# WUTCM-Lab/GLSDet

Hardware: AMD Instinct MI355X
Metric: images/sec fwd @1333x800 bs=8 (detection forward incl. decode+NMS) (higher is better)
Workload: dtype f16; 1 GPU; yolox_s_glfusion_1344x800_bs8; detector=YOLOX-s + GL-fusion neck, images_per_gpu=8, global_batch=8, num_classes=10, hip_graph=True, batches_in_flight=3, parallelism=image-sharded dp1, one all_gather of detections per step

## Files before the change

### glsdet_amd/_lib.py

```python
import ctypes as C
import threading
import os

HERE = os.path.dirname(os.path.abspath(__file__))
LIB_PATH = os.path.join(HERE, "lib", "libglsdet_hip.so")
ABI_VERSION = 13
CAPTURE_LOCK = threading.RLock()

F16, F32 = 0, 1
ACT = {"none": 0, "silu": 1, "relu": 2, "lrelu": 3, "gelu": 4, "sigmoid": 5}


class GlsdetLibraryError(RuntimeError):
    pass


class GlsdetError(RuntimeError):
    """A C-ABI call returned a negative code; nothing was launched."""


class View(C.Structure):
    _fields_ = [("base", C.c_void_p), ("sn", C.c_int64), ("sh", C.c_int64), ("sw", C.c_int64),
                ("n", C.c_int32), ("h", C.c_int32), ("w", C.c_int32), ("c", C.c_int32),
                ("dtype", C.c_int32), ("_pad", C.c_int32),
                ("alloc_lo", C.c_void_p), ("alloc_hi", C.c_void_p)]


class ConvDesc(C.Structure):
    _fields_ = [("x", View), ("y", View), ("res", View),
                ("w", C.c_void_p), ("scale", C.c_void_p), ("bias", C.c_void_p),
                ("R", C.c_int32), ("S", C.c_int32), ("stride", C.c_int32), ("pad", C.c_int32),
                ("act", C.c_int32), ("tile_hint", C.c_int32)]


class ConvChain(C.Structure):
    _fields_ = [("y2", View), ("w2", C.c_void_p), ("scale2", C.c_void_p), ("bias2", C.c_void_p),
                ("act2", C.c_int32), ("c0", C.c_int32), ("cin2", C.c_int32), ("flags", C.c_int32)]


_SIGS = {
    "glsdet_conv2d_chain": (C.c_int, [C.POINTER(ConvDesc), C.POINTER(ConvChain), C.c_void_p]),
    "glsdet_conv2d_chain_tune": (C.c_int, [C.POINTER(ConvDesc), C.POINTER(ConvChain), C.c_void_p, C.POINTER(C.c_int32),
                                           C.POINTER(C.c_float)]),
    "glsdet_conv2d_gnstats_bytes": (C.c_int64, [C.c_int32, C.c_int32, C.c_int32, C.c_int32]),
    "glsdet_conv2d_gnstats": (C.c_int, [C.POINTER(ConvDesc), C.c_int32, C.c_void_p, C.c_void_p]),
    "glsdet_conv2d_gnstats_tune": (C.c_int, [C.POINTER(ConvDesc), C.c_int32, C.c_void_p, C.c_void_p, C.POINTER(C.c_int32),
                                             C.POINTER(C.c_float)]),
    "glsdet_bottleneck": (C.c_int, [C.POINTER(ConvDesc), C.POINTER(ConvDesc), C.c_int32, C.c_void_p]),
    "glsdet_bottleneck_tune": (C.c_int, [C.POINTER(ConvDesc), C.POINTER(ConvDesc), C.c_void_p, C.POINTER(C.c_int32),
                                         C.POINTER(C.c_float)]),
    "glsdet_conv2d": (C.c_int, [C.POINTER(ConvDesc), C.c_void_p]),
    "glsdet_conv2d_multi": (C.c_int, [C.POINTER(ConvDesc), C.c_int32, C.c_void_p]),
    "glsdet_conv2d_multi_tune": (C.c_int, [C.POINTER(ConvDesc), C.c_int32, C.c_void_p, C.POINTER(C.c_int32),
                                           C.POINTER(C.c_float)]),
    "glsdet_conv2d_tune": (C.c_int, [C.POINTER(ConvDesc), C.c_void_p, C.POINTER(C.c_int32), C.POINTER(C.c_float)]),
    "glsdet_dwconv2d": (C.c_int, [C.POINTER(ConvDesc), C.c_void_p]),
    "glsdet_dwconv2d_dilated": (C.c_int, [C.POINTER(ConvDesc), C.c_int32, C.c_void_p]),
    "glsdet_gate": (C.c_int, [C.POINTER(View), C.POINTER(View), C.POINTER(View), C.POINTER(View), C.c_int32, C.c_void_p]),
    "glsdet_conv_weight_elems": (C.c_int64, [C.c_int32] * 5),
    "glsdet_conv_kpad": (C.c_int32, [C.c_int32] * 4),
    "glsdet_conv_cout_pad": (C.c_int32, [C.c_int32]),
    "glsdet_focus_pack": (C.c_int, [C.c_void_p, C.c_int32, C.c_int32, C.c_int32, C.c_int32,
                                    C.POINTER(View), C.c_void_p]),
    "glsdet_focus_conv": (C.c_int, [C.c_void_p, C.c_int32, C.c_int32, C.c_int32, C.c_int32, C.c_void_p, C.c_void_p, C.c_void_p,
                                    C.c_int32, C.POINTER(View), C.c_void_p]),
    "glsdet_focus_conv_down": (C.c_int, [C.c_void_p, C.c_int32, C.c_int32, C.c_int32, C.c_int32, C.c_void_p, C.c_void_p, C.c_void_p,
                                         C.c_int32, C.c_int32, C.c_void_p, C.c_void_p, C.c_void_p, C.c_int32, C.POINTER(View),
                                         C.c_void_p]),
    "glsdet_resnet_stem_weight_elems": (C.c_int64, []),
    "glsdet_resnet_stem_pool": (C.c_int, [C.c_void_p, C.c_int32, C.c_int32, C.c_int32, C.c_int32, C.c_void_p, C.c_void_p, C.c_void_p,
                                          C.POINTER(View), C.c_void_p]),
    "glsdet_resnet_stem": (C.c_int, [C.c_void_p, C.c_int32, C.c_int32, C.c_int32, C.c_int32, C.c_void_p, C.c_void_p, C.c_void_p,
                                     C.c_int32, C.POINTER(View), C.c_void_p]),
    "glsdet_channel_maxmean": (C.c_int, [C.POINTER(View), C.POINTER(View), C.c_void_p]),
    "glsdet_spp_pools": (C.c_int, [C.POINTER(View), C.POINTER(View), C.POINTER(View), C.POINTER(View), C.c_void_p]),
    "glsdet_maxpool2d": (C.c_int, [C.POINTER(View), C.POINTER(View), C.c_int32, C.c_void_p]),
    "glsdet_resample_copy": (C.c_int, [C.POINTER(View), C.POINTER(View), C.c_int32, C.c_void_p]),
    "glsdet_copy_many": (C.c_int, [C.POINTER(View), C.POINTER(View), C.c_int32, C.c_void_p]),
    "glsdet_transpose_many": (C.c_int, [C.POINTER(View), C.POINTER(View), C.c_int32, C.c_void_p]),
    "glsdet_nonlocal": (C.c_int, [C.POINTER(View), C.POINTER(View), C.c_int32, C.c_void_p, C.c_void_p,
                                  C.c_void_p, C.POINTER(View), C.c_void_p]),
    "glsdet_nonlocal_multi": (C.c_int, [C.POINTER(View), C.POINTER(View), C.c_int32, C.c_int32, C.POINTER(C.c_void_p),
                                        C.POINTER(C.c_void_p), C.c_void_p, C.POINTER(View), C.c_void_p]),
    "glsdet_attn_split": (C.c_int, [C.POINTER(View), C.c_void_p, C.c_void_p]),
    "glsdet_nonlocal_split": (C.c_int, [C.POINTER(View), C.POINTER(View), C.c_int32, C.POINTER(C.c_void_p), C.POINTER(C.c_void_p),
                                        C.c_void_p, C.POINTER(View), C.c_void_p, C.c_int32, C.c_void_p]),
    "glsdet_rowsplit": (C.c_int, [C.POINTER(View), C.POINTER(View), C.POINTER(View), C.c_void_p, C.c_int32, C.c_void_p]),
    "glsdet_scale_by_map": (C.c_int, [C.POINTER(View), C.POINTER(View), C.POINTER(View), C.c_void_p]),
    "glsdet_yolox_decode": (C.c_int, [C.POINTER(View), C.c_int32, C.c_int32, C.c_int32, C.c_int32,
                                      C.POINTER(C.c_int32), C.c_int32, C.c_void_p, C.c_int64, C.c_void_p, C.c_void_p]),
    "glsdet_nms_workspace_bytes": (C.c_int64, [C.c_int32, C.c_int32, C.c_int32]),
    "glsdet_nms": (C.c_int, [C.c_void_p, C.c_int32, C.c_int32, C.c_int32, C.c_int32, C.c_float, C.c_float,
                             C.c_int32, C.c_int32, C.c_void_p, C.c_void_p, C.c_void_p, C.c_void_p,
# ... 89 lines not shown
```

### glsdet_amd/engine.py

```python
from __future__ import annotations

import ctypes as C
import json
import os
import threading
from typing import List, Optional, Sequence, Tuple

import numpy as np
import torch

from . import _lib
from ._lib import F16, F32, ACT, View, ConvChain, ConvDesc, check

_TORCH_DT = {F16: torch.float16, F32: torch.float32}
_ESIZE = {F16: 2, F32: 4}


def ceil_to(v: int, m: int) -> int:
    return (v + m - 1) // m * m


class TView:
    __slots__ = ("buf", "off", "n", "h", "w", "c", "sn", "sh", "sw", "dtype")

# ... 251 lines not shown
            ref = self.tensor(out2.n, out2.h, out2.w, out2.c, out2.dtype)
            self.conv(out.channels(c0, c0 + cin2), packed2, 1, 0, act2, out=ref, tile_hint=1)
            a, b = out2.to_nchw(), ref.to_nchw()
            self.shadow["log"].append({"shape": (x.n, out.h, out.w, cin2, out2.c, 1, 1), "scale": float(a.abs().max()),
                                       "err": float((a - b).abs().max()), "nan": bool(torch.isnan(a).any()),
                                       "differ": float((a != b).float().mean())})
        return ok

    def bottleneck(self, x: TView, packed1, act1: str, packed2, act2: str, out: TView, res: Optional[TView],
                   hidden: TView) -> bool:
        w1, s1, b1, cm, R1, S1 = packed1
        w2, s2, b2, cout, R2, S2 = packed2
        if (R1, S1, R2, S2) != (1, 1, 3, 3) or cm != cout or cm not in (32, 64, 128) or x.dtype != out.dtype:
            return False
        hid = hidden
        d1, d2 = ConvDesc(), ConvDesc()
        d1.x, d1.y, d1.res = x.as_c(), hid.as_c(), View()
        d1.w, d1.scale, d1.bias = w1.data_ptr(), s1.data_ptr(), b1.data_ptr()
        d1.R, d1.S, d1.stride, d1.pad, d1.act, d1.tile_hint = 1, 1, 1, 0, ACT[act1], 0
        d2.x, d2.y = hid.as_c(), out.as_c()
        d2.res = res.as_c() if res is not None else View()
        d2.w, d2.scale, d2.bias = w2.data_ptr(), s2.data_ptr(), b2.data_ptr()
        d2.R, d2.S, d2.stride, d2.pad, d2.act, d2.tile_hint = 3, 3, 1, 1, ACT[act2], 0
        st = _stream_ptr(self.stream)
        hint = 0
        if self.autotune:
            key = ("bneck", x.n, x.h, x.w, x.c, x.sn, x.sh, x.sw, cm, out.sn, out.sh, out.sw, res is not None, out.dtype)
            if key not in self._tuned:
                best, us = C.c_int32(0), C.c_float(0)
                hint = best.value if self.lib.glsdet_bottleneck_tune(C.byref(d1), C.byref(d2), st, C.byref(best), C.byref(us)) == 0 else -1
                if hint >= 0:
                    hint = best.value
                    h1, u1, h2, u2 = C.c_int32(0), C.c_float(0), C.c_int32(0), C.c_float(0)
                    if self.lib.glsdet_conv2d_tune(C.byref(d1), st, C.byref(h1), C.byref(u1)) == 0 and \
                            self.lib.glsdet_conv2d_tune(C.byref(d2), st, C.byref(h2), C.byref(u2)) == 0 and \
                            us.value > 0.97 * (u1.value + u2.value) + _fuse_credit_us() and not os.environ.get("GLSDET_FORCE_BNECK"):
                        hint = -1
                self._tuned[key] = hint
                self._tune_dirty = True
            hint = self._tuned[key]
            if hint < 0:
                return False
        ok = self.lib.glsdet_bottleneck(C.byref(d1), C.byref(d2), hint, st) == 0
        if ok and self.shadow is not None:
            ref = self.tensor(out.n, out.h, out.w, out.c, out.dtype)
            self.conv(x, packed1, 1, 0, act1, out=hidden, tile_hint=1)
            self.conv(hidden, packed2, 1, 1, act2, out=ref, res=res, tile_hint=1)
            a, b = out.to_nchw(), ref.to_nchw()
            self.shadow["log"].append({"shape": (x.n, out.h, out.w, cm, cm, 3, 3), "scale": float(a.abs().max()),
                                       "err": float((a - b).abs().max()), "nan": bool(torch.isnan(a).any()),
                                       "differ": float((a != b).float().mean())})
        return ok

    def conv_multi(self, xs: Sequence[TView], packs, stride: int, pad: int, act: str,
                   outs: Optional[Sequence[Optional[TView]]] = None, ress: Optional[Sequence[Optional[TView]]] = None,
                   out_dtype: Optional[int] = None, tile_hint: int = 0) -> List[TView]:
        n = len(xs)
        assert 1 <= n <= 32 and len(packs) == n
        outs = list(outs) if outs is not None else [None] * n
        ress = list(ress) if ress is not None else [None] * n
        arr = (ConvDesc * n)()
        for i, (x, pk) in enumerate(zip(xs, packs)):
            wdev, sdev, bdev, cout, R, S = pk
            if outs[i] is None:
                outs[i] = self.tensor(x.n, (x.h + 2 * pad - R) // stride + 1, (x.w + 2 * pad - S) // stride + 1, cout, out_dtype)
            d = arr[i]
            d.x, d.y = x.as_c(), outs[i].as_c()
            d.res = ress[i].as_c() if ress[i] is not None else View()
            d.w, d.scale, d.bias = wdev.data_ptr(), sdev.data_ptr(), bdev.data_ptr()
            d.R, d.S, d.stride, d.pad, d.act, d.tile_hint = R, S, stride, pad, ACT[act], tile_hint
        sh = None
        if self.shadow is not None and self.shadow.get("multi"):
            sh = self._shadow_begin([arr[i] for i in range(n)], outs, self.shadow["multi"], multi=True)
        forced = os.environ.get("GLSDET_FORCE_MULTI_HINT")
        if forced and tile_hint == 0:
            arr[0].tile_hint = int(forced, 0)
            if self.lib.glsdet_conv2d_multi(arr, n, _stream_ptr(self.stream)) == 0:
                return outs
            arr[0].tile_hint = 0
        check(self.lib.glsdet_conv2d_multi(arr, n, _stream_ptr(self.stream)), "conv2d_multi")
        self._shadow_end(sh)
        return outs

    def conv_many(self, xs: Sequence[TView], packs, stride: int, pad: int, act: str, outs: Sequence[TView],
                  ress: Optional[Sequence[Optional[TView]]] = None) -> List[TView]:
        ress = list(ress) if ress is not None else [None] * len(xs)
        n = len(xs)
        geo = lambda x, pk, o, r: (x.n, x.h, x.w, x.c, x.sn, x.sh, x.sw, x.dtype, pk[3], pk[4], pk[5], o.n, o.h, o.w, o.c, o.sn, o.sh,
                                   o.sw, o.dtype) + ((-1, -1, -1, -1) if r is None else (r.sn, r.sh, r.sw, r.c))
        per = 8
        if n > 8 and stride == 1 and pad == 0 and packs[0][4] == 1 and packs[0][5] == 1 and not os.environ.get("GLSDET_NO_BATCH") and \
                len({geo(x, pk, o, r) for x, pk, o, r in zip(xs, packs, outs, ress)}) == 1:
            per = 32
        for i in range(0, n, per):
            k = min(per, n - i)
            hint = 0
            if k > 8 and self.autotune:
                key = ("batch", k, act) + geo(xs[i], packs[i], outs[i], ress[i])
                if key not in self._tuned:
                    arr = (ConvDesc * k)()
                    for j in range(k):
                        d, pk, r = arr[j], packs[i + j], ress[i + j]
                        d.x, d.y = xs[i + j].as_c(), outs[i + j].as_c()
                        d.res = r.as_c() if r is not None else View()
                        d.w, d.scale, d.bias = pk[0].data_ptr(), pk[1].data_ptr(), pk[2].data_ptr()
                        d.R, d.S, d.stride, d.pad, d.act, d.tile_hint = 1, 1, 1, 0, ACT[act], 0
# ... 485 lines not shown
```

### glsdet_amd/nets.py

```python
from __future__ import annotations

import os

from typing import Dict, List, Optional, Sequence

import torch

from ._lib import F32
from .engine import Engine, TView, ceil_to, fold_bn

BN_EPS = 1e-3


class NetBuilder:
    def __init__(self, eng: Engine, sd: Dict[str, torch.Tensor]):
        self.e = eng
        self.sd = {k: v.detach().cpu() for k, v in sd.items()}
        self._packed = {}
        self._override = {}
        self.trace = None
        self.composed = None

    def _rec(self, name: str, v: TView, c0: int = 0, c1: Optional[int] = None):
        if self.trace is not None:
# ... 80 lines not shown

    def plain(self, p: str, x: TView, pad: int = 0, out: Optional[TView] = None, act: str = "none",
              res: Optional[TView] = None) -> TView:
        pk = self._pack(p, [self._plain_part(p)], x.c)
        y = self.e.conv(x, pk, 1, pad, act, out=out, res=res)
        self._rec(p, y, 0, pk[3])
        return y

    def conv_out_channels(self, p: str) -> int:
        if self.is_depthwise(p):
            return self.sd[p + ".pconv.conv.weight"].shape[0]
        return self.sd[p + ".conv.weight"].shape[0]

    def _cba_chain(self, prefixes, x: TView, nxt: str, cin2: int, out: TView, res: Optional[TView] = None) -> Optional[TView]:
        if isinstance(prefixes, str):
            prefixes = [prefixes]
        if os.environ.get("GLSDET_NO_CHAIN") or any(self.is_depthwise(q) for q in list(prefixes) + [nxt]):
            return None
        parts = [self._bn_part(q) for q in prefixes]
        k = parts[0][0].shape[-1]
        pk = self._pack("+".join(prefixes), parts, x.c)
        w2 = self.sd[nxt + ".conv.weight"]
        if w2.shape[-1] != 1 or w2.shape[1] != cin2:
            return None
        pk2 = self._pack(nxt, [self._bn_part(nxt)], cin2)
        t = self.e.tensor(x.n, out.h, out.w, w2.shape[0])
        if not self.e.conv_chain(x, pk, 1, (k - 1) // 2, "silu", out, res, pk2, "silu", 0, cin2, t):
            return None
        c0 = 0
        for q, pt in zip(prefixes, parts):
            self._rec(q, out, c0, c0 + pt[0].shape[0])
            c0 += pt[0].shape[0]
        self._rec(nxt, t, 0, w2.shape[0])
        return t

    def _csp_entry(self, prefixes, x: Optional[TView], dst: TView, down):
        if down is not None:
            dp, dx = down
            cin2 = self.conv_out_channels(dp)
            hid2 = sum(self.conv_out_channels(q) for q in prefixes)
            ok = False
            if not os.environ.get("GLSDET_NO_DOWN_CHAIN") and not os.environ.get("GLSDET_NO_CHAIN") and hid2 <= 128 and \
                    not any(self.is_depthwise(q) for q in list(prefixes) + [dp]):
                pk = self._pack(dp, [self._bn_part(dp)], dx.c)
                pk2 = self._pack("+".join(prefixes), [self._bn_part(q) for q in prefixes], ceil_to(cin2, 8))
                ho, wo = (dx.h + 2 - 3) // 2 + 1, (dx.w + 2 - 3) // 2 + 1
                scratch = self.e.tensor(dx.n, ho, wo, cin2)
                ok = self.e.conv_chain(dx, pk, 2, 1, "silu", scratch, None, pk2, "silu", 0, scratch.c, dst, skip_y=True)
            if ok:
                return
            x = self.cba(dp, dx, 2)
        self.cba(list(prefixes), x, out=dst)

    def csp(self, p: str, x: Optional[TView], shortcut: bool, out: Optional[TView] = None, down=None) -> TView:
        hid = self.conv_out_channels(p + ".conv1")
        n = 0
        while self.has("%s.m.%d.conv1.conv.weight" % (p, n)):
            n += 1
        if n and hid in (32, 64, 128) and not os.environ.get("GLSDET_NO_BNECK_FUSION") and self.trace is None and \
                not self.is_depthwise("%s.m.0.conv2" % p) and self.sd["%s.m.0.conv2.conv.weight" % p].shape[-1] == 3:
            if x is None:
                dn, dh, dw = down[1].n, (down[1].h + 2 - 3) // 2 + 1, (down[1].w + 2 - 3) // 2 + 1
            else:
                dn, dh, dw = x.n, x.h, x.w
            buf = self.e.tensor(dn, dh, dw, 3 * hid)
            P, Q = buf.channels(0, hid), buf.channels(2 * hid, 3 * hid)
            scratch = self.e.tensor(dn, dh, dw, hid)
            cur, oth = (P, Q) if n % 2 == 0 else (Q, P)
            probe = lambda i, src, dst: self.e.bottleneck(src, self._pack("%s.m.%d.conv1" % (p, i), [self._bn_part("%s.m.%d.conv1" % (p, i))], hid),
                                                          "silu", self._pack("%s.m.%d.conv2" % (p, i), [self._bn_part("%s.m.%d.conv2" % (p, i))], hid),
                                                          "silu", dst, src if shortcut else None, scratch)
            if n % 2 == 0:
                self._csp_entry([p + ".conv1", p + ".conv2"], x, buf.channels(0, 2 * hid), down)
            else:
                self._csp_entry([p + ".conv2", p + ".conv1"], x, buf.channels(hid, 3 * hid), down)
            for i in range(n):
                if not probe(i, cur, oth):
                    t = self.cba("%s.m.%d.conv1" % (p, i), cur, out=scratch)
                    self.cba("%s.m.%d.conv2" % (p, i), t, out=oth, res=cur if shortcut else None)
                else:
                    self._rec("%s.m.%d.conv2" % (p, i), oth, 0, hid)
                cur, oth = oth, cur
            return self.cba(p + ".conv3", buf.channels(0, 2 * hid), out=out)
        if x is None and down is not None and not (self.trace is None and 2 * hid <= 128):
            x, down = self.cba(down[0], down[1], 2), None
        if x is None:
            cat = self.e.tensor(down[1].n, (down[1].h + 2 - 3) // 2 + 1, (down[1].w + 2 - 3) // 2 + 1, 2 * hid)
            self._csp_entry([p + ".conv1", p + ".conv2"], None, cat, down)
            t = None
        else:
            cat = self.e.tensor(x.n, x.h, x.w, 2 * hid)
            t = self._cba_chain([p + ".conv1", p + ".conv2"], x, "%s.m.0.conv1" % p, hid, cat) if n else None
            if t is None:
                self.cba([p + ".conv1", p + ".conv2"], x, out=cat)
        a = cat.channels(0, hid)
        for i in range(n):
            if t is None:
                t = self.cba("%s.m.%d.conv1" % (p, i), a)
            t_next = None
            if i + 1 < n:
                t_next = self._cba_chain("%s.m.%d.conv2" % (p, i), t, "%s.m.%d.conv1" % (p, i + 1), hid, a,
                                         res=a if shortcut else None)
            if t_next is None:
                self.cba("%s.m.%d.conv2" % (p, i), t, out=a, res=a if shortcut else None)
            t = t_next
        return self.cba(p + ".conv3", cat, out=out)

    def spp(self, p: str, x: TView, out: Optional[TView] = None) -> TView:
        hid = self.conv_out_channels(p + ".conv1")
        cat = self.e.tensor(x.n, x.h, x.w, 4 * hid)
        self.cba(p + ".conv1", x, out=cat.channels(0, hid))
        if os.environ.get("GLSDET_NO_SPP_FUSION"):
            for i in range(3):
                self.e.maxpool(cat.channels(i * hid, (i + 1) * hid), 5, out=cat.channels((i + 1) * hid, (i + 2) * hid))
        else:
            self.e.spp_pools(cat.channels(0, hid), cat.channels(hid, 2 * hid), cat.channels(2 * hid, 3 * hid), cat.channels(3 * hid, 4 * hid))
        return self.cba(p + ".conv2", cat, out=out)

    def darknet(self, p: str, img: torch.Tensor, homes: Dict[str, Optional[TView]]) -> Dict[str, TView]:
        f = {}
        q = p + ".stem.conv"
        w0 = self.sd.get(q + ".conv.weight")
        d2 = p + ".dark2.0"
        wd = self.sd.get(d2 + ".conv.weight")
        fused_down = False
        if w0 is not None and img.shape[1] == 3 and tuple(w0.shape[1:]) == (12, 3, 3) and w0.shape[0] <= 64 and \
                not os.environ.get("GLSDET_NO_STEM_FUSION"):
            if w0.shape[0] == 32 and wd is not None and tuple(wd.shape[1:]) == (32, 3, 3) and wd.shape[0] <= 64 and self.trace is None \
                    and img.shape[2] % 4 == 0 and img.shape[3] % 4 == 0 and os.environ.get("GLSDET_STEM2_FUSION"):
                x = self.e.focus_conv_down(img, self._pack(q, [self._bn_part(q)], 16), "silu", self._pack(d2, [self._bn_part(d2)], 32), "silu")
                fused_down = True
            else:
                x = self.e.focus_conv(img, self._pack(q, [self._bn_part(q)], 16), "silu")
                self._rec(q, x, 0, w0.shape[0])
        else:
            x = self.cba(q, self.e.focus_pack(img))
        att = lambda i: self.has("%s.lsk%d.proj_1.weight" % (p, i))
        for i, name in enumerate(("dark2", "dark3", "dark4")):
            down = None
            if not (fused_down and name == "dark2"):
                d0 = "%s.%s.0" % (p, name)
                if self.trace is None and not self.is_depthwise(d0) and 2 * self.conv_out_channels("%s.%s.1.conv1" % (p, name)) <= 128 \
                        and self.sd[d0 + ".conv.weight"].shape[-1] == 3:
                    down = (d0, x)
                    x = None
                else:
                    x = self.cba(d0, x, 2)
            if att(i + 2):
                x = self.csp("%s.%s.1" % (p, name), x, True, down=down)
                x = self.attention("%s.lsk%d" % (p, i + 2), x, out=homes.get(name))
            else:
                x = self.csp("%s.%s.1" % (p, name), x, True, out=homes.get(name), down=down)
            f[name] = x
        x = self.cba(p + ".dark5.0", x, 2)
        x = self.spp(p + ".dark5.1", x)
        if att(5):
            x = self.csp(p + ".dark5.2", x, False)
            x = self.attention(p + ".lsk5", x, out=homes.get("dark5"))
        else:
            x = self.csp(p + ".dark5.2", x, False, out=homes.get("dark5"))
        f["dark5"] = x
        return f

    def nonlocal_block(self, p: str, x: TView) -> TView:
        ci = self.sd[p + ".theta.weight"].shape[0]
        key = p + ".tpg"
        parts = [self._plain_part(p + ".theta"), self._plain_part(p + ".phi"), self._plain_part(p + ".g")]
        tpg = self.e.conv(x, self._pack(key, parts, x.c), 1, 0, "none")
        for j, nm in enumerate(("theta", "phi", "g")):
            self._rec("%s.%s" % (p, nm), tpg, j * ci, (j + 1) * ci)
        if key + ".out" not in self._packed:
            w = self.sd[p + ".conv_out.weight"].float().reshape(-1, ci)
            self._packed[key + ".out"] = (self.e.upload(w), self.e.upload(self.sd[p + ".conv_out.bias"].float()))
        wout, bout = self._packed[key + ".out"]
        assert wout.shape[0] == x.c, "Non_local_Block conv_out must map back to the input channels"
        y = self.e.nonlocal_(x, tpg, ci, wout, bout, out=x)
        self._rec(p + ".conv_out", y)
        return y

    def nonlocal_blocks(self, ps: Sequence[str], xs: Sequence[TView]) -> List[TView]:
        ci = self.sd[ps[0] + ".theta.weight"].shape[0]
        packs = []
        for p, x in zip(ps, xs):
            parts = [self._plain_part(p + ".theta"), self._plain_part(p + ".phi"), self._plain_part(p + ".g")]
            packs.append(self._pack(p + ".tpg", parts, x.c))
        tpgs = self.e.conv_group(xs, packs, 1, 0, "none")
        for p, tpg in zip(ps, tpgs):
            for j, nm in enumerate(("theta", "phi", "g")):
                self._rec("%s.%s" % (p, nm), tpg, j * ci, (j + 1) * ci)
        wouts, bouts = [], []
        for p, x in zip(ps, xs):
            key = p + ".tpg"
            if key + ".out" not in self._packed:
                w = self.sd[p + ".conv_out.weight"].float().reshape(-1, ci)
                self._packed[key + ".out"] = (self.e.upload(w), self.e.upload(self.sd[p + ".conv_out.bias"].float()))
            wout, bout = self._packed[key + ".out"]
            assert wout.shape[0] == x.c, "Non_local_Block conv_out must map back to the input channels"
            wouts.append(wout)
            bouts.append(bout)
        if len({(x.n, x.c) for x in xs}) == 1 and len(xs) <= 4 and not os.environ.get("GLSDET_NO_GROUP"):
            ys = self.e.nonlocal_multi(xs, tpgs, ci, wouts, bouts)
        else:
            ys = [self.e.nonlocal_(x, tpg, ci, w, b, out=x) for x, tpg, w, b in zip(xs, tpgs, wouts, bouts)]
        for p, y in zip(ps, ys):
            self._rec(p + ".conv_out", y)
        return ys

    def compose_1x1_input(self, consumer: str, c0: int, c1: int, lin: str):
        w, s, b = self._bn_part(consumer)
        wl = self.sd[lin + ".weight"].double().reshape(self.sd[lin + ".weight"].shape[0], -1)
        bl = self.sd[lin + ".bias"].double()
        W = w.double().reshape(w.shape[0], -1)
        assert W.shape[1] >= c1 and c1 - c0 == wl.shape[0]
# ... 343 lines not shown
```

### include/glsdet_hip.h

```cpp
#ifndef GLSDET_HIP_H
#define GLSDET_HIP_H

#include <stdint.h>

#ifdef __cplusplus
extern "C" {
#endif

#define GLSDET_ABI_VERSION 13

enum { GLSDET_F16 = 0, GLSDET_F32 = 1 };
enum { GLSDET_ACT_NONE = 0, GLSDET_ACT_SILU = 1, GLSDET_ACT_RELU = 2, GLSDET_ACT_LRELU = 3,
       GLSDET_ACT_GELU = 4 , GLSDET_ACT_SIGMOID = 5,
       GLSDET_ACT_RES_FIRST = 0x100 };
enum {
  GLSDET_OK = 0,
  GLSDET_E_ARG = -1,
  GLSDET_E_BOUNDS = -2,
  GLSDET_E_ALIGN = -3,
  GLSDET_E_HIP = -4,
  GLSDET_E_CAPACITY = -5
};

typedef struct glsdet_view {
  void*   base;
  int64_t sn, sh, sw;
  int32_t n, h, w, c;
  int32_t dtype;
  int32_t _pad;
  void*   alloc_lo;
  void*   alloc_hi;
} glsdet_view;

typedef struct glsdet_conv_desc {
  glsdet_view x, y, res;
  const void*  w;
  const float* scale;
  const float* bias;
  int32_t R, S, stride, pad, act;
  int32_t tile_hint;
} glsdet_conv_desc;

int     glsdet_conv2d(const glsdet_conv_desc* d, void* stream);
int     glsdet_conv2d_multi(const glsdet_conv_desc* d, int32_t n, void* stream);
int     glsdet_conv2d_multi_tune(const glsdet_conv_desc* d, int32_t n, void* stream, int32_t* best_hint, float* best_us);
int     glsdet_conv2d_tune(const glsdet_conv_desc* d, void* stream, int32_t* best_hint, float* best_us);
typedef struct glsdet_conv_chain {
  glsdet_view y2;
  const void*  w2;
  const float* scale2;
  const float* bias2;
  int32_t act2, c0, cin2;
  int32_t flags;
} glsdet_conv_chain;
#define GLSDET_CHAIN_SKIP_Y 1
int     glsdet_conv2d_chain(const glsdet_conv_desc* d, const glsdet_conv_chain* c, void* stream);
int     glsdet_conv2d_chain_tune(const glsdet_conv_desc* d, const glsdet_conv_chain* c, void* stream, int32_t* best_hint,
                                 float* best_us);
int     glsdet_bottleneck(const glsdet_conv_desc* c1, const glsdet_conv_desc* c2, int32_t hint, void* stream);
int     glsdet_bottleneck_tune(const glsdet_conv_desc* c1, const glsdet_conv_desc* c2, void* stream, int32_t* best_hint,
                               float* best_us);
int     glsdet_dwconv2d(const glsdet_conv_desc* d, void* stream);
int     glsdet_dwconv2d_dilated(const glsdet_conv_desc* d, int32_t dilation, void* stream);
int64_t glsdet_conv_weight_elems(int32_t cout, int32_t R, int32_t S, int32_t cin, int32_t dtype);
int32_t glsdet_conv_kpad(int32_t R, int32_t S, int32_t cin, int32_t dtype);
int32_t glsdet_conv_cout_pad(int32_t cout);

int glsdet_focus_pack(const float* img, int32_t n, int32_t cin, int32_t H, int32_t W,
                      const glsdet_view* y, void* stream);

int glsdet_focus_conv(const float* img, int32_t n, int32_t cin, int32_t H, int32_t W, const void* w, const float* scale,
                      const float* bias, int32_t act, const glsdet_view* y, void* stream);
int glsdet_focus_conv_down(const float* img, int32_t n, int32_t cin, int32_t H, int32_t W, const void* w1, const float* scale1,
                           const float* bias1, int32_t act1, int32_t c1, const void* w2, const float* scale2,
                           const float* bias2, int32_t act2, const glsdet_view* y, void* stream);

int glsdet_maxpool2d(const glsdet_view* x, const glsdet_view* y, int32_t k, void* stream);

int glsdet_spp_pools(const glsdet_view* x, const glsdet_view* y5, const glsdet_view* y9, const glsdet_view* y13, void* stream);

int glsdet_channel_maxmean(const glsdet_view* x, const glsdet_view* y, void* stream);

int glsdet_resample_copy(const glsdet_view* x, const glsdet_view* y, int32_t factor, void* stream);

int glsdet_copy_many(const glsdet_view* x, const glsdet_view* y, int32_t count, void* stream);

int glsdet_transpose_many(const glsdet_view* x, const glsdet_view* y, int32_t count, void* stream);

int glsdet_nonlocal(const glsdet_view* x, const glsdet_view* tpg, int32_t ci,
                    const float* wout, const float* bout, float* gram,
                    const glsdet_view* out, void* stream);
int glsdet_nonlocal_multi(const glsdet_view* x, const glsdet_view* tpg, int32_t n_sets, int32_t ci,
                          const float* const* wout, const float* const* bout, float* gram,
                          const glsdet_view* out, void* stream);

int glsdet_attn_split(const glsdet_view* att, int32_t* split, void* stream);
int glsdet_nonlocal_split(const glsdet_view* x, const glsdet_view* tpg , int32_t ci, const float* const* wout ,
                          const float* const* bout , float* gram, const glsdet_view* out, const int32_t* split,
                          int32_t split_shift , void* stream);
int glsdet_rowsplit(const glsdet_view* a, const glsdet_view* b , const glsdet_view* y, const int32_t* split, int32_t mode,
                    void* stream);
int glsdet_scale_by_map(const glsdet_view* x, const glsdet_view* map, const glsdet_view* y, void* stream);

int glsdet_yolox_decode(const glsdet_view* levels, int32_t n_levels, int32_t num_classes,
                        int32_t in_h, int32_t in_w, const int32_t* strides ,
                        int32_t mode, float* out, int64_t out_elems,
                        const float* scale_factors, void* stream);

int64_t glsdet_nms_workspace_bytes(int32_t n, int32_t A, int32_t max_cand);
int glsdet_nms(const float* pred, int32_t n, int32_t A, int32_t num_classes, int32_t box_mode,
               float conf_thres, float nms_thres, int32_t max_cand, int32_t max_det,
               float* dets, int32_t* count, int32_t* status,
               void* ws, int64_t ws_bytes, void* stream);

// ... 95 lines not shown
```

Measured before the change: 4622 img/s.

## Fuse whole 64-channel CSP block into one tiled HIP kernel

Adds a kernel that runs an entire CSP layer (conv1+conv2 1x1, bottleneck 1x1 and 3x3 with shortcut, conv3 1x1) per spatial tile, keeping intermediates in LDS and reusing weights across a strip of tiles. It targets the 64->64, hidden-32, single-bottleneck CSP stages of the backbone. The aim is to cut the global-memory round trips and launches of the separate convs and bottleneck kernels. Autotuning keeps the fused path only when it times under the unfused sequence. The cost is large LDS use with limited occupancy and recomputation of the halo ring.

```diff
diff --git a/glsdet_amd/_lib.py b/glsdet_amd/_lib.py
--- a/glsdet_amd/_lib.py
+++ b/glsdet_amd/_lib.py
@@ -4,7 +4,7 @@
 
 HERE = os.path.dirname(os.path.abspath(__file__))
 LIB_PATH = os.path.join(HERE, "lib", "libglsdet_hip.so")
-ABI_VERSION = 13
+ABI_VERSION = 14
 CAPTURE_LOCK = threading.RLock()
 
 F16, F32 = 0, 1
@@ -38,7 +38,15 @@
                 ("act2", C.c_int32), ("c0", C.c_int32), ("cin2", C.c_int32), ("flags", C.c_int32)]
 
 
+class CspDesc(C.Structure):
+    _fields_ = [("x", View), ("y", View)] + \
+               [(k + q, C.c_void_p) for q in ("12", "m1", "m2", "3") for k in ("w", "scale", "bias")] + \
+               [("act", C.c_int32), ("shortcut", C.c_int32)]
+
+
 _SIGS = {
+    "glsdet_csp_fused": (C.c_int, [C.POINTER(CspDesc), C.c_int32, C.c_void_p]),
+    "glsdet_csp_fused_tune": (C.c_int, [C.POINTER(CspDesc), C.c_void_p, C.POINTER(C.c_int32), C.POINTER(C.c_float)]),
     "glsdet_conv2d_chain": (C.c_int, [C.POINTER(ConvDesc), C.POINTER(ConvChain), C.c_void_p]),
     "glsdet_conv2d_chain_tune": (C.c_int, [C.POINTER(ConvDesc), C.POINTER(ConvChain), C.c_void_p, C.POINTER(C.c_int32),
                                            C.POINTER(C.c_float)]),
diff --git a/glsdet_amd/csrc/conv_csp.hip b/glsdet_amd/csrc/conv_csp.hip
--- /dev/null
+++ b/glsdet_amd/csrc/conv_csp.hip
@@ -0,0 +1,405 @@
+#include "conv_common.h"
+
+namespace glsdet {
+
+struct CspArgs {
+  const unsigned char* x_lo;
+  unsigned x_off, x_bytes;
+  long x_sn, x_sh, x_sw;
+  unsigned char* y_lo;
+  unsigned y_off, y_bytes;
+  long y_sn, y_sh, y_sw;
+  const unsigned char *w12, *wm1, *wm2, *w3;
+  const float *s12, *b12, *sm1, *bm1, *sm2, *bm2, *s3, *b3;
+  int N, H, W, shortcut;
+  int kp12, kpm1, kpm2, kp3;
+  int tiles_x, tiles_y, strips_x, strip;
+};
+
+template <int TH>
+struct CspGeom {
+  static constexpr int PW = 18, PH = TH + 2, NSLOT = PH * PW;
+  static constexpr int NHB = (NSLOT + 31) / 32, NS32 = NHB * 32;
+  static constexpr int NPX = TH * 16, NIB = NPX / 32;
+  static constexpr int RS = 64 * 2 + 16;
+  static constexpr int RSH = 32 * 2 + 16;
+  static constexpr int RSW = 9 * 32 * 2 + 16;
+  static constexpr int WM1_OFF = 0, WM2_OFF = WM1_OFF + 32 * RSH, SB_OFF = WM2_OFF + 32 * RSW;
+  static constexpr int R1_OFF = SB_OFF + 384 * 4;
+  static constexpr int R2_OFF = R1_OFF + NS32 * RS;
+  static constexpr int LDS = R2_OFF + NS32 * RS;
+  static constexpr int S12 = 0, B12 = 64, S3 = 128, B3 = 192, SM1 = 256, BM1 = 288, SM2 = 320, BM2 = 352;
+};
+
+template <int TH>
+__global__ __launch_bounds__(256, 2) void csp_fused_kernel(const CspArgs a) {
+  using G = CspGeom<TH>;
+  using T = f16;
+  constexpr int PW = G::PW, NSLOT = G::NSLOT, NHB = G::NHB, NIB = G::NIB, RS = G::RS, RSH = G::RSH, RSW = G::RSW;
+  extern __shared__ __attribute__((aligned(16))) unsigned char smem[];
+  unsigned char* sWm1 = smem + G::WM1_OFF;
+  unsigned char* sWm2 = smem + G::WM2_OFF;
+  const float* sSB = reinterpret_cast<const float*>(smem + G::SB_OFF);
+  unsigned char* sR1 = smem + G::R1_OFF;
+  unsigned char* sMS = smem + G::R2_OFF;
+  const int tid = threadIdx.x, lane = tid & 63, l31 = lane & 31, lh = lane >> 5;
+  const int wave = __builtin_amdgcn_readfirstlane(tid >> 6);
+
+  int t;
+  {
+    const int nwg = gridDim.x, bid = blockIdx.x;
+    const int q = nwg >> 3, r = nwg & 7, xcd = bid & 7, local = bid >> 3;
+    t = (xcd < r ? xcd * (q + 1) : r * (q + 1) + (xcd - r) * q) + local;
+  }
+  const int sx = t % a.strips_x;
+  t /= a.strips_x;
+  const int ty = t % a.tiles_y, img = t / a.tiles_y;
+  const int ty0 = ty * TH;
+
+  const auto xrs = gls_make_rsrc(a.x_lo, a.x_bytes);
+  const auto yrs = gls_make_rsrc(a.y_lo, a.y_bytes);
+  constexpr int NP = G::NS32 / 32;
+  const int kc = tid & 7, slot0 = tid >> 3;
+  u32x4 pre[NP];
+  auto issue_loads = [&](int tx0) __attribute__((always_inline)) {
+#pragma unroll
+    for (int i = 0; i < NP; ++i) {
+      const int slot = slot0 + i * 32;
+      const int py = slot / PW, px = slot - py * PW;
+      const int hi = ty0 - 1 + py, wi = tx0 - 1 + px;
+      const bool ok = slot < NSLOT && (unsigned)hi < (unsigned)a.H && (unsigned)wi < (unsigned)a.W;
+      const unsigned off = ok ? a.x_off + (unsigned)(((long)img * a.x_sn + (long)hi * a.x_sh + (long)wi * a.x_sw + kc * 8) * 2L) : GLS_OOB;
+      pre[i] = gls_buf_load16(xrs, off);
+    }
+  };
+  issue_loads(sx * a.strip * 16);
+
+  for (int q = tid; q < 32 * 4; q += 256) {
+    const int row = q >> 2, c = q & 3;
+    *reinterpret_cast<u32x4*>(sWm1 + row * RSH + c * 16) = *reinterpret_cast<const u32x4*>(a.wm1 + (long)row * a.kpm1 * 2 + c * 16);
+  }
+  for (int q = tid; q < 32 * 36; q += 256) {
+    const int row = q / 36, c = q - row * 36;
+    *reinterpret_cast<u32x4*>(sWm2 + row * RSW + c * 16) = *reinterpret_cast<const u32x4*>(a.wm2 + (long)row * a.kpm2 * 2 + c * 16);
+  }
+  if (tid < 96) {
+    const float* src;
+    int j;
+    if (tid < 64) {
+      j = tid & 15;
+      src = tid < 16 ? a.s12 : (tid < 32 ? a.b12 : (tid < 48 ? a.s3 : a.b3));
+    } else {
+      j = tid & 7;
+      const int k = (tid - 64) >> 3;
+      src = k == 0 ? a.sm1 : (k == 1 ? a.bm1 : (k == 2 ? a.sm2 : a.bm2));
+    }
+    *reinterpret_cast<f32x4*>(smem + G::SB_OFF + tid * 16) = *reinterpret_cast<const f32x4*>(src + j * 4);
+  }
+  constexpr int NI1 = 2 * NHB / 4, NI4 = 2 * NIB / 4;
+  static_assert((2 * NHB) % 4 == 0 && (2 * NIB) % 4 == 0, "units per wave");
+  u32x4 a12[4], a3[NI4][4];
+#pragma unroll
+  for (int kk = 0; kk < 4; ++kk)
+    a12[kk] = *reinterpret_cast<const u32x4*>(a.w12 + (long)((wave & 1) * 32 + l31) * a.kp12 * 2 + kk * 32 + lh * 16);
+#pragma unroll
+  for (int i = 0; i < NI4; ++i)
+#pragma unroll
+    for (int kk = 0; kk < 4; ++kk)
+      a3[i][kk] = *reinterpret_cast<const u32x4*>(a.w3 + (long)(((wave + 4 * i) / NIB) * 32 + l31) * a.kp3 * 2 + kk * 32 + lh * 16);
+#pragma unroll
+  for (int kk = 0; kk < 4; ++kk) asm volatile("" ::"v"(a12[kk]));
+#pragma unroll
+  for (int i = 0; i < NI4; ++i)
+#pragma unroll
+    for (int kk = 0; kk < 4; ++kk) asm volatile("" ::"v"(a3[i][kk]));
+
+  for (int s = 0; s < a.strip; ++s) {
+    const int tx = sx * a.strip + s;
+    if (tx >= a.tiles_x) break;
+    const int tx0 = tx * 16;
+    __syncthreads();
+#pragma unroll
+    for (int i = 0; i < NP; ++i) *reinterpret_cast<u32x4*>(sR1 + (slot0 + i * 32) * RS + kc * 16) = pre[i];
+    if (s + 1 < a.strip && tx + 1 < a.tiles_x) issue_loads(tx0 + 16);
+    __syncthreads();
+
+    {
+      f32x16 acc[NI1];
+#pragma unroll
+      for (int i = 0; i < NI1; ++i)
+#pragma unroll
+        for (int e = 0; e < 16; ++e) acc[i][e] = 0.0f;
+      const int cb = wave & 1, pb0 = wave >> 1;
+#pragma unroll
+      for (int kk = 0; kk < 4; ++kk)
+#pragma unroll
+        for (int i = 0; i < NI1; ++i) {
+          const u32x4 bf = *reinterpret_cast<const u32x4*>(sR1 + ((pb0 + 2 * i) * 32 + l31) * RS + kk * 32 + lh * 16);
+          MMA<T>::run(a12[kk], bf, acc[i]);
+        }
+#pragma unroll
+      for (int i = 0; i < NI1; ++i) {
+        const int p = (pb0 + 2 * i) * 32 + l31;
+#pragma unroll
+        for (int g = 0; g < 4; ++g) {
+          const int co = cb * 32 + 8 * g + 4 * lh;
+          const f32x4 sc = *reinterpret_cast<const f32x4*>(sSB + G::S12 + co), bi = *reinterpret_cast<const f32x4*>(sSB + G::B12 + co);
+          const f32x4 xv = {acc[i][4 * g], acc[i][4 * g + 1], acc[i][4 * g + 2], acc[i][4 * g + 3]};
+          const f32x4 yv = scale_bias_act4<T>(xv, sc, bi, GLSDET_ACT_SILU);
+          const float v[4] = {yv[0], yv[1], yv[2], yv[3]};
+          store4(sMS + p * RS + co * 2, v, (T*)nullptr);
+        }
+      }
+    }
+    __syncthreads();
+
+#pragma unroll
+    for (int i = 0; i < (NHB + 3) / 4; ++i) {
+      const int pb = wave + 4 * i;
+      if (pb < NHB) {
+        f32x16 acc;
+#pragma unroll
+        for (int e = 0; e < 16; ++e) acc[e] = 0.0f;
+        const int p = pb * 32 + l31;
+#pragma unroll
+        for (int kk = 0; kk < 2; ++kk) {
+          const u32x4 af = *reinterpret_cast<const u32x4*>(sWm1 + l31 * RSH + kk * 32 + lh * 16);
+          const u32x4 bf = *reinterpret_cast<const u32x4*>(sMS + p * RS + kk * 32 + lh * 16);
+          MMA<T>::run(af, bf, acc);
+        }
+        const int py = p / PW, px = p - py * PW;
+        const int hi = ty0 - 1 + py, wi = tx0 - 1 + px;
+        const bool inside = (unsigned)hi < (unsigned)a.H && (unsigned)wi < (unsigned)a.W;
+#pragma unroll
+        for (int g = 0; g < 4; ++g) {
+          const int co = 8 * g + 4 * lh;
+          const f32x4 sc = *reinterpret_cast<const f32x4*>(sSB + G::SM1 + co), bi = *reinterpret_cast<const f32x4*>(sSB + G::BM1 + co);
+          const f32x4 xv = {acc[4 * g], acc[4 * g + 1], acc[4 * g + 2], acc[4 * g + 3]};
+          f32x4 yv = scale_bias_act4<T>(xv, sc, bi, GLSDET_ACT_SILU);
+          if (!inside) yv = f32x4{0.f, 0.f, 0.f, 0.f};
+          const float v[4] = {yv[0], yv[1], yv[2], yv[3]};
+          store4(sR1 + p * RSH + co * 2, v, (T*)nullptr);
+        }
+      }
+    }
+    __syncthreads();
+
+    if (wave < NIB) {
+      f32x16 acc;
+#pragma unroll
+      for (int e = 0; e < 16; ++e) acc[e] = 0.0f;
+      int oy, ox;
+      pix_to_xy16<PW>(wave * 32 + l31, oy, ox);
+      const unsigned char* brow = sR1 + (oy * PW + ox) * RSH + lh * 16;
+      const unsigned char* arow = sWm2 + l31 * RSW + lh * 16;
+#pragma unroll
+      for (int tap = 0; tap < 9; ++tap)
+#pragma unroll
+        for (int kk = 0; kk < 2; ++kk) {
+          const u32x4 af = *reinterpret_cast<const u32x4*>(arow + tap * 64 + kk * 32);
+          const u32x4 bf = *reinterpret_cast<const u32x4*>(brow + ((tap / 3) * PW + tap % 3) * RSH + kk * 32);
+          MMA<T>::run(af, bf, acc);
+        }
+      unsigned char* mrow = sMS + ((oy + 1) * PW + ox + 1) * RS;
+#pragma unroll
+      for (int g = 0; g < 4; ++g) {
+        const int co = 8 * g + 4 * lh;
+        const f32x4 sc = *reinterpret_cast<const f32x4*>(sSB + G::SM2 + co), bi = *reinterpret_cast<const f32x4*>(sSB + G::BM2 + co);
+        const f32x4 xv = {acc[4 * g], acc[4 * g + 1], acc[4 * g + 2], acc[4 * g + 3]};
+        const f32x4 yv = scale_bias_act4<T>(xv, sc, bi, GLSDET_ACT_SILU);
+        float v[4] = {yv[0], yv[1], yv[2], yv[3]};
+        if (a.shortcut) {
+          const f16x4 m = *reinterpret_cast<const f16x4*>(mrow + co * 2);
+#pragma unroll
+          for (int e = 0; e < 4; ++e) {
+            asm volatile("" : "+v"(v[e]));
+            v[e] = v[e] + (float)m[e];
+          }
+        }
+        store4(mrow + co * 2, v, (T*)nullptr);
+      }
+    }
+    __syncthreads();
+
+    {
+      f32x16 acc[NI4];
+#pragma unroll
+      for (int i = 0; i < NI4; ++i)
+#pragma unroll
+        for (int e = 0; e < 16; ++e) acc[i][e] = 0.0f;
+      int pn[NI4];
+#pragma unroll
+      for (int i = 0; i < NI4; ++i) {
+        const int u = wave + 4 * i;
+        int oy, ox;
+        pix_to_xy16<PW>((u % NIB) * 32 + l31, oy, ox);
+        pn[i] = oy * 16 + ox;
+        const unsigned char* brow = sMS + ((oy + 1) * PW + ox + 1) * RS + lh * 16;
+#pragma unroll
+        for (int kk = 0; kk < 4; ++kk) {
+          const u32x4 bf = *reinterpret_cast<const u32x4*>(brow + kk * 32);
+          MMA<T>::run(a3[i][kk], bf, acc[i]);
+        }
+      }
+#pragma unroll
+      for (int i = 0; i < NI4; ++i) {
+        const int cb = (wave + 4 * i) / NIB;
+#pragma unroll
+        for (int g = 0; g < 4; ++g) {
+          const int co = cb * 32 + 8 * g + 4 * lh;
+          const f32x4 sc = *reinterpret_cast<const f32x4*>(sSB + G::S3 + co), bi = *reinterpret_cast<const f32x4*>(sSB + G::B3 + co);
+          const f32x4 xv = {acc[i][4 * g], acc[i][4 * g + 1], acc[i][4 * g + 2], acc[i][4 * g + 3]};
+          const f32x4 yv = scale_bias_act4<T>(xv, sc, bi, GLSDET_ACT_SILU);
+          const float v[4] = {yv[0], yv[1], yv[2], yv[3]};
+          store4(sR1 + pn[i] * RS + co * 2, v, (T*)nullptr);
+        }
+      }
+    }
+    __syncthreads();
+#pragma unroll
+    for (int k = 0; k < G::NPX * 8 / 256; ++k) {
+      const int q = tid + k * 256;
+      const int px_l = q >> 3, cq = q & 7;
+      const int ho = ty0 + (px_l >> 4), wo = tx0 + (px_l & 15);
+      const bool ok = ho < a.H && wo < a.W;
+      const unsigned off = ok ? a.y_off + (unsigned)(((long)img * a.y_sn + (long)ho * a.y_sh + (long)wo * a.y_sw + cq * 8) * 2L) : GLS_OOB;
+      __builtin_amdgcn_raw_buffer_store_b128(*reinterpret_cast<const u32x4*>(sR1 + px_l * RS + cq * 16), yrs, (int)off, 0, 0);
+    }
+  }
+}
+
+template <int TH>
+static int launch_csp(const CspArgs& a0, hipStream_t st) {
+  using G = CspGeom<TH>;
+  auto kern = csp_fused_kernel<TH>;
+  static bool attr_set = false;
+  if (!attr_set && G::LDS > 64 * 1024) {
+    GLS_HIP(hipFuncSetAttribute(reinterpret_cast<const void*>(kern), hipFuncAttributeMaxDynamicSharedMemorySize, G::LDS));
+    attr_set = true;
+  }
+  CspArgs a = a0;
+  a.tiles_x = (a.W + 15) / 16;
+  a.tiles_y = (a.H + TH - 1) / TH;
+  const long rows = (long)a.N * a.tiles_y;
+  int best = 1;
+  long best_cost = -1;
+  for (int sl = 1; sl <= 8 && sl <= a.tiles_x; ++sl) {
+    const long wgs = rows * ((a.tiles_x + sl - 1) / sl);
+    const long cost = ((wgs + 511) / 512) * (sl + 1);
+    if (best_cost < 0 || cost <= best_cost) { best = sl; best_cost = cost; }
+  }
+  a.strip = best;
+  a.strips_x = (a.tiles_x + a.strip - 1) / a.strip;
+  const long grid = rows * a.strips_x;
+  if (grid <= 0 || grid > 0x7fffffffL) GLS_FAIL(GLSDET_E_ARG, "csp_fused: grid %ld out of range", grid);
+  hipLaunchKernelGGL(kern, dim3((unsigned)grid), dim3(256), G::LDS, st, a);
+  GLS_HIP(hipGetLastError());
+  return 0;
+}
+
+static int build_csp_op(const glsdet_csp_desc* d, int hint, OpRecord& op) {
+  if (!d) GLS_FAIL(GLSDET_E_ARG, "csp_fused: null descriptor");
+  const glsdet_view &x = d->x, &y = d->y;
+  int rc;
+  if ((rc = check_view(x, "csp_fused.x"))) return rc;
+  if ((rc = check_view(y, "csp_fused.y"))) return rc;
+  if (x.dtype != GLSDET_F16 || y.dtype != GLSDET_F16) GLS_FAIL(GLSDET_E_ARG, "csp_fused: fp16 storage only");
+  if (x.c != 64 || y.c != 64) GLS_FAIL(GLSDET_E_ARG, "csp_fused: 64 -> 64 channels (hidden 32, one Bottleneck) only, got %d -> %d", x.c, y.c);
+  if (y.n != x.n || y.h != x.h || y.w != x.w) GLS_FAIL(GLSDET_E_ARG, "csp_fused: output extent [%d,%d,%d] != input [%d,%d,%d]", y.n, y.h, y.w, x.n, x.h, x.w);
+  const void* ptrs[12] = {d->w12, d->scale12, d->bias12, d->wm1, d->scalem1, d->biasm1, d->wm2, d->scalem2, d->biasm2, d->w3, d->scale3, d->bias3};
+  for (const void* p : ptrs) {
+    if (!p) GLS_FAIL(GLSDET_E_ARG, "csp_fused: null weight/scale/bias");
+    if ((uintptr_t)p & 15) GLS_FAIL(GLSDET_E_ALIGN, "csp_fused: weight/scale/bias must be 16-byte aligned");
+  }
+  if (d->act != GLSDET_ACT_SILU) GLS_FAIL(GLSDET_E_ARG, "csp_fused: act %d, only SiLU (BaseConv's) is compiled", d->act);
+  if (d->shortcut != 0 && d->shortcut != 1) GLS_FAIL(GLSDET_E_ARG, "csp_fused: shortcut must be 0 or 1");
+  if (hint != 0 && hint != 1) GLS_FAIL(GLSDET_E_ARG, "csp_fused: hint must be 0 (8 x 16 tiles) or 1 (4 x 16)");
+  const long M = (long)x.n * x.h * x.w;
+  if (M <= 0 || M > 0x7fffffffL) GLS_FAIL(GLSDET_E_ARG, "csp_fused: pixel count %ld out of range", M);
+  const int64_t xalloc = (const char*)x.alloc_hi - (const char*)x.alloc_lo;
+  const int64_t yalloc = (const char*)y.alloc_hi - (const char*)y.alloc_lo;
+  if (xalloc >= 0x7fffffffLL || yalloc >= 0x7fffffffLL)
+    GLS_FAIL(GLSDET_E_ARG, "csp_fused: operand allocation of %lld bytes exceeds the 2 GiB descriptor range", (long long)(xalloc > yalloc ? xalloc : yalloc));
+  const char *xlo = (const char*)x.base, *ylo = (const char*)y.base;
+  const int64_t xspan = ((int64_t)(x.n - 1) * x.sn + (int64_t)(x.h - 1) * x.sh + (int64_t)(x.w - 1) * x.sw + x.c) * 2;
+  const int64_t yspan = ((int64_t)(y.n - 1) * y.sn + (int64_t)(y.h - 1) * y.sh + (int64_t)(y.w - 1) * y.sw + y.c) * 2;
+  if (xlo < ylo + yspan && ylo < xlo + xspan) {
+    const bool same_geom = x.sn == y.sn && x.sh == y.sh && x.sw == y.sw;
+    const int64_t dd = (ylo - xlo) / 2, sw = x.sw;
+    const bool disjoint = same_geom && (dd > 0 ? (dd >= x.c && dd + y.c <= sw) : (dd < 0 && -dd >= y.c && -dd + x.c <= sw));
+    if (!disjoint) GLS_FAIL(GLSDET_E_ARG, "csp_fused: y overlaps x (the fused form cannot run in place)");
+  }
+  CspArgs a = {};
+  a.x_lo = (const unsigned char*)x.alloc_lo;
+  a.x_off = (unsigned)((const char*)x.base - (const char*)x.alloc_lo);
+  a.x_bytes = (unsigned)xalloc;
+  a.x_sn = x.sn; a.x_sh = x.sh; a.x_sw = x.sw;
+  a.y_lo = (unsigned char*)y.alloc_lo;
+  a.y_off = (unsigned)((const char*)y.base - (const char*)y.alloc_lo);
+  a.y_bytes = (unsigned)yalloc;
+  a.y_sn = y.sn; a.y_sh = y.sh; a.y_sw = y.sw;
+  a.w12 = (const unsigned char*)d->w12; a.s12 = d->scale12; a.b12 = d->bias12;
+  a.wm1 = (const unsigned char*)d->wm1; a.sm1 = d->scalem1; a.bm1 = d->biasm1;
+  a.wm2 = (const unsigned char*)d->wm2; a.sm2 = d->scalem2; a.bm2 = d->biasm2;
+  a.w3 = (const unsigned char*)d->w3; a.s3 = d->scale3; a.b3 = d->bias3;
+  a.N = x.n; a.H = x.h; a.W = x.w; a.shortcut = d->shortcut;
+  a.kp12 = a.kp3 = glsdet_conv_kpad(1, 1, 64, GLSDET_F16);
+  a.kpm1 = glsdet_conv_kpad(1, 1, 32, GLSDET_F16);
+  a.kpm2 = glsdet_conv_kpad(3, 3, 32, GLSDET_F16);
+  op.kind = 0;
+  op.flops = 2.0 * (double)M * (64.0 * 64 + 32.0 * 32 + 32.0 * 288 + 64.0 * 64);
+  op.bytes = 2.0 * (double)M * 64 * 2;
+  char nm[112];
+  snprintf(nm, sizeof nm, "csp_fused<f16,32,%dx16> 64->64 hid32 3x3%s", hint ? 4 : 8, d->shortcut ? " +x" : "");
+  op.name = nm;
+  op.launch = [a, hint](hipStream_t st) -> int { return hint ? launch_csp<4>(a, st) : launch_csp<8>(a, st); };
+  return 0;
+}
+
+}
+
+using namespace glsdet;
+
+extern "C" int glsdet_csp_fused(const glsdet_csp_desc* d, int32_t hint, void* stream) {
+  OpRecord op;
+  int rc = build_csp_op(d, hint, op);
+  if (rc) return rc;
+  return submit(std::move(op), stream);
+}
+
+extern "C" int glsdet_csp_fused_tune(const glsdet_csp_desc* d, void* stream, int32_t* best_hint, float* best_us) {
+  if (!best_hint) GLS_FAIL(GLSDET_E_ARG, "csp_fused_tune: null argument");
+  OpRecord ops[2];
+  for (int h = 0; h < 2; ++h) {
+    int rc = build_csp_op(d, h, ops[h]);
+    if (rc) return rc;
+  }
+  hipStream_t st = (hipStream_t)stream;
+  for (int h = 0; h < 2; ++h) {
+    int rc = ops[h].launch(st);
+    if (rc) return rc;
+  }
+  constexpr int TRIALS = 3, REPS = 5;
+  hipEvent_t e0, e1;
+  GLS_HIP(hipEventCreate(&e0));
+  GLS_HIP(hipEventCreate(&e1));
+  float us[2] = {1e30f, 1e30f};
+  int rc = 0;
+  for (int t = 0; t < TRIALS && !rc; ++t)
+    for (int h = 0; h < 2 && !rc; ++h) {
+      (void)hipEventRecord(e0, st);
+      for (int r = 0; r < REPS && !rc; ++r) rc = ops[h].launch(st);
+      (void)hipEventRecord(e1, st);
+      if (hipEventSynchronize(e1) != hipSuccess) rc = GLSDET_E_HIP;
+      float ms = 0.f;
+      (void)hipEventElapsedTime(&ms, e0, e1);
+      if (!rc && ms * 1000.f / REPS < us[h]) us[h] = ms * 1000.f / REPS;
+    }
+  (void)hipEventDestroy(e0);
+  (void)hipEventDestroy(e1);
+  if (rc) GLS_FAIL(rc, "csp_fused_tune: a timed launch failed");
+  *best_hint = us[1] < us[0] ? 1 : 0;
+  if (best_us) *best_us = us[*best_hint];
+  set_error("");
+  return 0;
+}
diff --git a/glsdet_amd/engine.py b/glsdet_amd/engine.py
--- a/glsdet_amd/engine.py
+++ b/glsdet_amd/engine.py
@@ -327,6 +327,83 @@
                                        "differ": float((a != b).float().mean())})
         return ok
 
+    def _tmp(self, n: int, h: int, w: int, c: int, sn: Optional[int] = None, sh: Optional[int] = None,
+             sw: Optional[int] = None) -> TView:
+        sw = c if sw is None else sw
+        sh = w * sw if sh is None else sh
+        sn = h * sh if sn is None else sn
+        buf = torch.zeros(ceil_to(n * sn * _ESIZE[self.dt], 256), dtype=torch.uint8, device=self.device)
+        return TView(buf, 0, n, h, w, c, sn, sh, sw, self.dt)
+
+    def _csp_desc(self, x: TView, out: TView, packs, shortcut: bool) -> "_lib.CspDesc":
+        d = _lib.CspDesc()
+        d.x, d.y = x.as_c(), out.as_c()
+        for q, pk in zip(("12", "m1", "m2", "3"), packs):
+            setattr(d, "w" + q, pk[0].data_ptr())
+            setattr(d, "scale" + q, pk[1].data_ptr())
+            setattr(d, "bias" + q, pk[2].data_ptr())
+        d.act, d.shortcut = ACT["silu"], 1 if shortcut else 0
+        return d
+
+    def _csp_unfused(self, x: TView, packs, shortcut: bool, out: TView, launch) -> None:
+        cat = self._tmp(x.n, x.h, x.w, 64)
+        t = self._tmp(x.n, x.h, x.w, 32)
+        main = cat.channels(0, 32)
+        launch(x, packs[0], 0, cat, None)
+        launch(main, packs[1], 0, t, None)
+        launch(t, packs[2], 1, main, main if shortcut else None)
+        launch(cat, packs[3], 0, out, None)
+
+    def csp_fused_wins(self, xg, og, packs, shortcut: bool) -> bool:
+        if self.dt != F16 or xg[3] != 64 or og[3] != 64 or tuple(xg[:3]) != tuple(og[:3]) or len(packs) != 4 or \
+                [(pk[3], pk[4], pk[5]) for pk in packs] != [(64, 1, 1), (32, 1, 1), (32, 3, 3), (64, 1, 1)]:
+            return False
+        if not self.autotune:
+            return True
+        key = ("csp1",) + tuple(int(v) for v in xg) + tuple(int(v) for v in og) + (bool(shortcut), int(self.dt))
+        if key not in self._tuned:
+            x, out = self._tmp(*xg), self._tmp(*og)
+            st = _stream_ptr(self.stream)
+            d = self._csp_desc(x, out, packs, shortcut)
+            best, us = C.c_int32(0), C.c_float(0)
+            hint = best.value if self.lib.glsdet_csp_fused_tune(C.byref(d), st, C.byref(best), C.byref(us)) == 0 else -1
+            if hint >= 0:
+                sep = []
+
+                def tune(xi, pk, pad, o, res):
+                    dd = ConvDesc()
+                    dd.x, dd.y = xi.as_c(), o.as_c()
+                    dd.res = res.as_c() if res is not None else View()
+                    dd.w, dd.scale, dd.bias = pk[0].data_ptr(), pk[1].data_ptr(), pk[2].data_ptr()
+                    dd.R, dd.S, dd.stride, dd.pad, dd.act, dd.tile_hint = pk[4], pk[5], 1, pad, ACT["silu"], 0
+                    b, u = C.c_int32(0), C.c_float(0)
+                    sep.append(u.value if self.lib.glsdet_conv2d_tune(C.byref(dd), st, C.byref(b), C.byref(u)) == 0 else None)
+
+                self._csp_unfused(x, packs, shortcut, out, tune)
+                if None not in sep and us.value > 0.97 * sum(sep) + _fuse_credit_us():
+                    hint = -1
+            self._tuned[key] = hint
+            self._tune_dirty = True
+        return self._tuned[key] >= 0
+
+    def csp_fused(self, x: TView, packs, shortcut: bool, out: TView) -> bool:
+        hint = 0
+        if self.autotune:
+            key = ("csp1", x.n, x.h, x.w, x.c, x.sn, x.sh, x.sw, out.n, out.h, out.w, out.c, out.sn, out.sh, out.sw,
+                   bool(shortcut), int(self.dt))
+            hint = max(self._tuned.get(key, 0), 0)
+        d = self._csp_desc(x, out, packs, shortcut)
+        ok = self.lib.glsdet_csp_fused(C.byref(d), hint, _stream_ptr(self.stream)) == 0
+        if ok and self.shadow is not None:
+            ref = self._tmp(out.n, out.h, out.w, out.c)
+            self._csp_unfused(x, packs, shortcut, ref,
+                              lambda xi, pk, pad, o, res: self.conv(xi, pk, 1, pad, "silu", out=o, res=res, tile_hint=1))
+            a, b = out.to_nchw(), ref.to_nchw()
+            self.shadow["log"].append({"shape": (x.n, out.h, out.w, 64, 64, 3, 3), "scale": float(a.abs().max()),
+                                       "err": float((a - b).abs().max()), "nan": bool(torch.isnan(a).any()),
+                                       "differ": float((a != b).float().mean())})
+        return ok
+
     def conv_multi(self, xs: Sequence[TView], packs, stride: int, pad: int, act: str,
                    outs: Optional[Sequence[Optional[TView]]] = None, ress: Optional[Sequence[Optional[TView]]] = None,
                    out_dtype: Optional[int] = None, tile_hint: int = 0) -> List[TView]:
diff --git a/glsdet_amd/nets.py b/glsdet_amd/nets.py
--- a/glsdet_amd/nets.py
+++ b/glsdet_amd/nets.py
@@ -156,11 +156,46 @@
             x = self.cba(dp, dx, 2)
         self.cba(list(prefixes), x, out=dst)
 
-    def csp(self, p: str, x: Optional[TView], shortcut: bool, out: Optional[TView] = None, down=None) -> TView:
+    def _csp_whole(self, p: str, x: Optional[TView], shortcut: bool, out: Optional[TView], down, hid: int, n: int):
+        if self.trace is not None or self.e.dt == F32 or hid != 32 or n != 1 or os.environ.get("GLSDET_NO_CSP_FUSION"):
+            return None, x, down
+        names = [p + ".conv1", p + ".conv2", p + ".m.0.conv1", p + ".m.0.conv2", p + ".conv3"]
+        if any(self.is_depthwise(q) for q in names) or self.sd[names[3] + ".conv.weight"].shape[-1] != 3 or \
+                self.sd[names[0] + ".conv.weight"].shape[1] != 64 or self.conv_out_channels(names[4]) != 64:
+            return None, x, down
+        if x is None:
+            dx = down[1]
+            dn, dh, dw = dx.n, (dx.h + 2 - 3) // 2 + 1, (dx.w + 2 - 3) // 2 + 1
+            xg = (dn, dh, dw, 64, dh * dw * 64, dw * 64, 64)
+        else:
+            dn, dh, dw = x.n, x.h, x.w
+            xg = (x.n, x.h, x.w, x.c, x.sn, x.sh, x.sw)
+        og = (dn, dh, dw, 64, dh * dw * 64, dw * 64, 64) if out is None else (out.n, out.h, out.w, out.c, out.sn, out.sh, out.sw)
+        packs = [self._pack(names[0] + "+" + names[1], [self._bn_part(names[0]), self._bn_part(names[1])], 64),
+                 self._pack(names[2], [self._bn_part(names[2])], 32), self._pack(names[3], [self._bn_part(names[3])], 32),
+                 self._pack(names[4], [self._bn_part(names[4])], 64)]
+        if not self.e.csp_fused_wins(xg, og, packs, shortcut):
+            return None, x, down
+        if x is None:
+            pk = self._pack(down[0], [self._bn_part(down[0])], down[1].c)
+            x = self.e.conv(down[1], pk, 2, 1, "silu", tile_hint=0 if self.e.autotune else 1)
+            self._rec(down[0], x, 0, pk[3])
+            down = None
+        y = out if out is not None else self.e.tensor(dn, dh, dw, 64)
+        if not self.e.csp_fused(x, packs, shortcut, y):
+            return None, x, down
+        self._rec(names[4], y, 0, 64)
+        return y, x, down
+
+    def csp(self, p: str, x: Optional[TView], shortcut: bool, out: Optional[TView] = None, down=None, whole: bool = False) -> TView:
         hid = self.conv_out_channels(p + ".conv1")
         n = 0
         while self.has("%s.m.%d.conv1.conv.weight" % (p, n)):
             n += 1
+        if whole:
+            y, x, down = self._csp_whole(p, x, shortcut, out, down, hid, n)
+            if y is not None:
+                return y
         if n and hid in (32, 64, 128) and not os.environ.get("GLSDET_NO_BNECK_FUSION") and self.trace is None and \
                 not self.is_depthwise("%s.m.0.conv2" % p) and self.sd["%s.m.0.conv2.conv.weight" % p].shape[-1] == 3:
             if x is None:
@@ -251,18 +286,18 @@
                 else:
                     x = self.cba(d0, x, 2)
             if att(i + 2):
-                x = self.csp("%s.%s.1" % (p, name), x, True, down=down)
+                x = self.csp("%s.%s.1" % (p, name), x, True, down=down, whole=True)
                 x = self.attention("%s.lsk%d" % (p, i + 2), x, out=homes.get(name))
             else:
-                x = self.csp("%s.%s.1" % (p, name), x, True, out=homes.get(name), down=down)
+                x = self.csp("%s.%s.1" % (p, name), x, True, out=homes.get(name), down=down, whole=True)
             f[name] = x
         x = self.cba(p + ".dark5.0", x, 2)
         x = self.spp(p + ".dark5.1", x)
         if att(5):
-            x = self.csp(p + ".dark5.2", x, False)
+            x = self.csp(p + ".dark5.2", x, False, whole=True)
             x = self.attention(p + ".lsk5", x, out=homes.get("dark5"))
         else:
-            x = self.csp(p + ".dark5.2", x, False, out=homes.get("dark5"))
+            x = self.csp(p + ".dark5.2", x, False, out=homes.get("dark5"), whole=True)
         f["dark5"] = x
         return f
 
diff --git a/include/glsdet_hip.h b/include/glsdet_hip.h
--- a/include/glsdet_hip.h
+++ b/include/glsdet_hip.h
@@ -7,7 +7,7 @@
 extern "C" {
 #endif
 
-#define GLSDET_ABI_VERSION 13
+#define GLSDET_ABI_VERSION 14
 
 enum { GLSDET_F16 = 0, GLSDET_F32 = 1 };
 enum { GLSDET_ACT_NONE = 0, GLSDET_ACT_SILU = 1, GLSDET_ACT_RELU = 2, GLSDET_ACT_LRELU = 3,
@@ -60,6 +60,17 @@
 int     glsdet_bottleneck(const glsdet_conv_desc* c1, const glsdet_conv_desc* c2, int32_t hint, void* stream);
 int     glsdet_bottleneck_tune(const glsdet_conv_desc* c1, const glsdet_conv_desc* c2, void* stream, int32_t* best_hint,
                                float* best_us);
+typedef struct glsdet_csp_desc {
+  glsdet_view x, y;
+  const void*  w12;  const float* scale12; const float* bias12;
+  const void*  wm1;  const float* scalem1; const float* biasm1;
+  const void*  wm2;  const float* scalem2; const float* biasm2;
+  const void*  w3;   const float* scale3;  const float* bias3;
+  int32_t act;
+  int32_t shortcut;
+} glsdet_csp_desc;
+int     glsdet_csp_fused(const glsdet_csp_desc* d, int32_t hint, void* stream);
+int     glsdet_csp_fused_tune(const glsdet_csp_desc* d, void* stream, int32_t* best_hint, float* best_us);
 int     glsdet_dwconv2d(const glsdet_conv_desc* d, void* stream);
 int     glsdet_dwconv2d_dilated(const glsdet_conv_desc* d, int32_t dilation, void* stream);
 int64_t glsdet_conv_weight_elems(int32_t cout, int32_t R, int32_t S, int32_t cin, int32_t dtype);
```

Measured after the change: 4788 img/s (median of 6 runs). 1.04x the previous value.
